# erizmr/SPH_Taichi

Measured on AMD Instinct MI355X. Metric: WCSPH steps/sec at 1.74 M particles (+ ms/step breakdown sort/neighbour/force), higher is better.
Workload: dtype f32

## Files before the change

### include/sph_hip.h

```cpp
#ifndef SPH_HIP_H
#define SPH_HIP_H

#include <stddef.h>
#include <stdint.h>

#ifdef __cplusplus
extern "C" {
#endif

#define SPH_ABI_VERSION 6

typedef struct SphContext SphContext;

typedef struct SphParams {
    int32_t n_particles;
    int32_t capacity;
    int32_t grid_num[3];
    int32_t cell_origin[3];
    int32_t n_objects;
    int32_t cold_capacity;
    float grid_size;
    float support_radius;
    float particle_diameter;
    float m_V0;
// ... 49 lines not shown
    SPH_OPT_FUSED_STEP = 2,
    SPH_OPT_BRICK_SHAPE = 3,
    SPH_OPT_NO_DYNAMIC_SOLIDS = 4 ,
    SPH_OPT_DEBUG_ABLATE = 5,
    SPH_OPT_SLAB_DROP_OUTSIDE = 6 ,
    SPH_OPT_UNIFORM_FLUID = 7  ,
    SPH_OPT_UNIFORM_FLUID_STATE = 8 ,
    SPH_OPT_SORT_BY_PID = 9    ,
    SPH_OPT_KERNEL_VARIANT = 10 ,
    SPH_OPT_RIGID_BATCH = 11   ,
    SPH_OPT_DF_RUNAHEAD = 13,
    SPH_OPT_EXACT_MATH = 12    ,
    SPH_OPT_RIGID_SUMS_FROM_X0 = 14,
    SPH_OPT_PURE_FLUID_INSTANCE = 15 ,
    SPH_OPT_BRICK_RECORDS = 16 ,
    SPH_OPT_DF_FUSE_ERROR = 17
};
#define SPH_VAR_GROUPS 1
#define SPH_VAR_MFMA 32
#define SPH_VAR_GAT_LDS 2
#define SPH_VAR_GAT_LDS4 4
#define SPH_VAR_FORCE_BF 8
#define SPH_VAR_DEEP 16

typedef struct SphTimings {
    double sort_ms, neighbour_ms, force_ms, integrate_ms, halo_ms, total_ms;
    int64_t steps;
} SphTimings;

int32_t sph_abi_version(void);
int32_t sph_device_count(void);
// ... 154 lines not shown
```

### sph_taichi_amd/_lib.py

```python
from __future__ import annotations

import ctypes as C
import os

from . import build as _build

_F3 = C.c_float * 3
_I3 = C.c_int32 * 3


class SphParams(C.Structure):
    _fields_ = [
        ("n_particles", C.c_int32), ("capacity", C.c_int32), ("grid_num", _I3), ("cell_origin", _I3),
        ("n_objects", C.c_int32), ("cold_capacity", C.c_int32),
        ("grid_size", C.c_float), ("support_radius", C.c_float), ("particle_diameter", C.c_float),
        ("m_V0", C.c_float), ("density_0", C.c_float), ("stiffness", C.c_float), ("exponent", C.c_float),
        ("viscosity", C.c_float), ("surface_tension", C.c_float), ("dt", C.c_float),
        ("g", _F3), ("domain_size", _F3), ("padding", C.c_float), ("wall_hi", _F3),
        ("k_w", C.c_float), ("k_dw", C.c_float), ("visc_d_nu", C.c_float), ("visc_eps", C.c_float),
    ]


class SphTimings(C.Structure):
    _fields_ = [("sort_ms", C.c_double), ("neighbour_ms", C.c_double), ("force_ms", C.c_double),
# ... 20 lines not shown


class SphRenderParams(C.Structure):
    _fields_ = [("width", C.c_int32), ("height", C.c_int32), ("eye", _F3), ("lookat", _F3), ("up", _F3),
                ("fov_y_deg", C.c_float), ("radius", C.c_float), ("near_plane", C.c_float), ("light", _F3),
                ("ambient", C.c_float), ("background", C.c_uint8 * 3), ("draw_box", C.c_uint8),
                ("box_end", _F3), ("box_color", _F3)]


RENDER_MAX_INVISIBLE = 32

F_OBJECT_ID, F_X, F_X_0, F_V, F_ACCELERATION, F_M_V, F_M, F_DENSITY, F_PRESSURE, F_MATERIAL, F_COLOR, \
    F_IS_DYNAMIC, F_GRID_IDS, F_GRID_PARTICLES_NUM, F_PID, F_RIGID_REST_CM, F_DFSPH_FACTOR, F_DENSITY_ADV = range(18)
OPT_GATHER_IMPL, OPT_TIMING, OPT_FUSED_STEP, OPT_BRICK_SHAPE, OPT_NO_DYNAMIC_SOLIDS, OPT_DEBUG_ABLATE, \
    OPT_SLAB_DROP_OUTSIDE, OPT_UNIFORM_FLUID, OPT_UNIFORM_FLUID_STATE, OPT_SORT_BY_PID, OPT_KERNEL_VARIANT, \
    OPT_RIGID_BATCH, OPT_EXACT_MATH, OPT_DF_RUNAHEAD, OPT_RIGID_SUMS_FROM_X0, OPT_PURE_FLUID_INSTANCE, OPT_BRICK_RECORDS, OPT_DF_FUSE_ERROR = range(18)
VAR_GROUPS, VAR_GAT_LDS, VAR_GAT_LDS4, VAR_FORCE_BF, VAR_DEEP, VAR_MFMA = 1, 2, 4, 8, 16, 32
VAR_DEFAULT = VAR_GROUPS | VAR_FORCE_BF | VAR_DEEP

ABI_VERSION = 6

_ctx = C.c_void_p
SYMBOLS = [
    ("sph_abi_version", C.c_int32, []),
    ("sph_device_count", C.c_int32, []),
    ("sph_create", C.c_int32, [C.POINTER(SphParams), C.c_int32, C.c_void_p, C.POINTER(_ctx)]),
    ("sph_destroy", C.c_int32, [_ctx]),
    ("sph_last_error", C.c_char_p, [_ctx]),
    ("sph_set_option", C.c_int32, [_ctx, C.c_int32, C.c_int32]),
    ("sph_get_option", C.c_int32, [_ctx, C.c_int32, C.POINTER(C.c_int32)]),
    ("sph_set_params", C.c_int32, [_ctx, C.POINTER(SphParams)]),
# ... 152 lines not shown
```

### sph_taichi_amd/csrc/sph_api.hip

```cpp
#include <sched.h>
#include "sph_internal.h"

#define SCAN_TILE 2048

int sphk_init_pid(SphContext* c);
int sphk_build_dyn_list(SphContext* c);

static thread_local char g_err[256] = "";

int sph_fail(SphContext* c, int code, const char* what) {
    if (c) snprintf(c->err, sizeof(c->err), "%s", what);
    else snprintf(g_err, sizeof(g_err), "%s", what);
    return code;
}

DevView sph_view(const SphContext* c) {
    DevView d;
    const SphParams& p = c->p;
    d.N = c->N; d.G = c->G;
    d.nx = p.grid_num[0]; d.ny = p.grid_num[1]; d.nz = p.grid_num[2];
    d.tgt_lo = 0; d.tgt_hi = p.grid_num[0]; d.tgt_lo2 = d.tgt_hi2 = 0;
#ifdef SPH_PROFILE
    d.ablate = c->opt_ablate;
    d.prof_ts = (c->opt_ablate & (3 << 28)) ? reinterpret_cast<unsigned long long*>(c->stage) : nullptr;
// ... 5 lines not shown
    d.d2 = p.particle_diameter * p.particle_diameter;
    d.m_V0 = p.m_V0; d.rho0 = p.density_0; d.stiffness = p.stiffness; d.exponent = p.exponent;
    d.exp_int = (p.exponent >= 1.0f && p.exponent <= 32.0f && p.exponent == (float)(int)p.exponent) ? (int)p.exponent : 0;
    d.sigma = p.surface_tension; d.dt = p.dt;
    d.gx = p.g[0]; d.gy = p.g[1]; d.gz = p.g[2];
    d.pad = p.padding;
    d.k_w = p.k_w; d.k_dw = p.k_dw; d.visc_d_nu = p.visc_d_nu; d.visc_eps = p.visc_eps;
    d.w_zero = p.k_w * (6.0f * 0.0f - 6.0f * 0.0f + 1.0f);
    {
        const float q = p.particle_diameter / p.support_radius;
        if (q <= 0.5f) d.w_d = p.k_w * (6.0f * q * q * q - 6.0f * q * q + 1.0f);
        else if (q <= 1.0f) d.w_d = p.k_w * 2.0f * (1.0f - q) * (1.0f - q) * (1.0f - q);
        else d.w_d = 0.0f;
    }
    const int o = c->in_off;
    d.xm = c->xm[c->cur] + o; d.vf = c->vf[c->cur] + o; d.aux = c->aux[c->cur] + o; d.key = c->key[c->cur] + o;
    d.eos = c->eos; d.eos2 = reinterpret_cast<float2*>(c->eos); d.acc = c->acc + o; d.acc_fx = c->acc_fx + 3 * (size_t)o; d.cell_end = c->cell_end;
    d.x0_cold = c->x0_cold; d.rigid_rest_cm = c->rigid_rest_cm; d.polar_fb = c->dyn_count ? c->dyn_count + 3 : nullptr;
    d.m_eps = c->df.m_eps;
    d.stg = c->stg; d.gat = c->gat; d.kbuf = reinterpret_cast<float*>(c->gat);
    d.m_u = c->m_uniform; d.write_sg = 0; d.write_k = 0;
    d.whx = p.wall_hi[0]; d.why = p.wall_hi[1]; d.whz = p.wall_hi[2];
    d.fuse_advect = c->fuse_advect;
    d.df_bpart = c->df_collect ? c->df_bpart : nullptr;
    d.gate = (c->df_epoch && c->opt_df_runahead) ? c->df_gate : nullptr;
    d.gate_epoch = c->df_epoch;
    d.fx_scale = ldexp(1.0, c->rigid_fx_exp);
    d.store_acc = !(c->fuse_advect && c->skip_acc);
    d.rigid_from_x0 = 0;
    return d;
}

__global__ void k_read_layer_offsets(const int* __restrict__ cell_end, const int* __restrict__ layers, int n,
                                     int per_layer, int* __restrict__ out) {
    const int k = blockIdx.x * blockDim.x + threadIdx.x;
    if (k >= n) return;
    const int L = layers[k];
    out[k] = L > 0 ? cell_end[(size_t)L * per_layer - 1] : 0;
// ... 68 lines not shown
    c->tgt_layers[0] = c->tgt_layers[2] = 0;
    c->tgt_layers[1] = c->tgt_layers[3] = params->grid_num[0];
    c->opt_gather_impl = 1;
    c->opt_fused = 1;
    c->opt_timing = 0;
    c->timing_phase = 0;
    c->opt_brick_shape = 0;
    c->opt_rigid_batch = 1;
    c->opt_df_fuse_err = 1;
    c->df_collect = 0;
    c->opt_df_runahead = 0;
    c->opt_exact_math = 0;
    c->opt_rigid_x0 = 0;
    c->opt_pure_instance = 1;
    c->opt_brick_rec = 1;
    if (stream) { c->stream = (hipStream_t)stream; c->own_stream = false; }
    else {
        if (hipStreamCreateWithFlags(&c->stream, hipStreamNonBlocking) != hipSuccess) {
            delete c;
            return sph_fail(nullptr, SPH_E_NO_DEVICE, "hipStreamCreate failed");
        }
        c->own_stream = true;
    }
    const size_t cap = (size_t)c->cap;
    c->scan_blocks = (c->G + 1 + SCAN_TILE - 1) / SCAN_TILE;
    int rc = 0;
    for (int s = 0; s < 2 && !rc; ++s) {
        rc = rc ? rc : alloc_dev(c, (void**)&c->xm[s], cap * 16);
        rc = rc ? rc : alloc_dev(c, (void**)&c->vf[s], cap * 16);
        rc = rc ? rc : alloc_dev(c, (void**)&c->aux[s], cap * 16);
// ... 62 lines not shown
    for (int s = 0; s < SPH_MAX_TIMED_STEPS && !rc; ++s)
        for (int k = 0; k < 5 && !rc; ++k)
            if (hipEventCreate(&c->ev[s][k]) != hipSuccess) rc = SPH_E_NOMEM;
    if (!rc && hipStreamSynchronize(c->stream) != hipSuccess) rc = SPH_E_NO_DEVICE;
    if (rc) {
        snprintf(g_err, sizeof(g_err), "sph_create failed: %s", c->err);
        sph_destroy(c);
        return rc;
    }
    c->n_dyn_host = -1;
    c->rigid_fx_exp = 30;
    sph_invalidate_lists(c);
    c->opt_uniform = -1; c->uniform_state = -1; c->m_uniform = 0.0f;
    c->opt_variant = SPH_VAR_DEFAULT;
    if (const char* e = getenv("SPH_KERNEL_VARIANT")) { const int v = atoi(e) & 31; c->opt_variant = variant_mask_ok(v) ? v : SPH_VAR_DEFAULT; }
    memset(&c->df_stats, 0, sizeof(c->df_stats));
    c->df.enable_divergence_solver = 1; c->df.m_max_iterations_v = 100; c->df.m_max_iterations = 100;
    c->df.fluid_particle_num = 0; c->df.m_eps = 1e-5f; c->df.reserved_ = 0.0f; c->df.max_error_V = 0.1; c->df.max_error = 0.05;
    *out = c;
    return 0;
}

int32_t sph_destroy(SphContext* c) {
    if (!c) return 0;
    (void)hipSetDevice(c->device);
    if (c->stream) (void)hipStreamSynchronize(c->stream);
    void* ptrs[] = {c->xm[0], c->xm[1], c->vf[0], c->vf[1], c->aux[0], c->aux[1], c->key[0], c->key[1], c->eos, c->stg, c->gat, c->acc,
                    c->acc_tmp, c->cell_buf[0], c->cell_buf[1], c->rank_off, c->idx_unstable, c->scan_status, c->x0_cold, c->color_cold,
                    c->rigid_rest_cm, c->dyn_list, c->dyn_count, c->acc_fx, c->rigid_part, c->rigid_R, c->df_err, c->df_part, c->df_bpart, c->stage, c->glist, c->gcnt, c->brick_list, c->brick_count, c->brick_list2, c->brick_count2, c->brick_rec};
    for (void* p : ptrs) if (p) (void)hipFree(p);
// ... 16 lines not shown

int32_t sph_set_option(SphContext* c, int32_t option, int32_t value) {
    if (!c) return SPH_E_INVALID;
    switch (option) {
        case SPH_OPT_GATHER_IMPL: if (value < 0 || value > 1) return sph_fail(c, SPH_E_INVALID, "gather impl must be 0 or 1"); c->opt_gather_impl = value; c->uniform_state = -1; return 0;
        case SPH_OPT_TIMING: c->opt_timing = value > 0 ? value : 0; c->timing_phase = 0; return 0;
        case SPH_OPT_FUSED_STEP: c->opt_fused = value ? 1 : 0; return 0;
        case SPH_OPT_BRICK_SHAPE: if (value < 0 || value > 1) return sph_fail(c, SPH_E_INVALID, "brick shape must be 0 (adaptive height) or 1 (fixed 4x2x4)"); c->opt_brick_shape = value; sph_invalidate_lists(c); return 0;
        case SPH_OPT_NO_DYNAMIC_SOLIDS: c->opt_no_dynamic = value ? 1 : 0; c->n_dyn_host = -1; c->uniform_state = -1; return 0;
        case SPH_OPT_DEBUG_ABLATE:
#ifndef SPH_PROFILE
            if (value != 0) return sph_fail(c, SPH_E_INVALID, "section ablation exists only in the profiling build (python -m sph_taichi_amd.build --profile; bench.py --ablate loads it)");
#endif
            c->opt_ablate = value;
            return 0;
        case SPH_OPT_SLAB_DROP_OUTSIDE: c->opt_drop_outside = value ? 1 : 0; c->uniform_state = -1; return 0;
        case SPH_OPT_SORT_BY_PID: c->opt_sort_by_pid = value ? 1 : 0; return 0;
        case SPH_OPT_RIGID_BATCH: c->opt_rigid_batch = value ? 1 : 0; return 0;
        case SPH_OPT_EXACT_MATH: c->opt_exact_math = value ? 1 : 0; sph_invalidate_lists(c); return 0;
        case SPH_OPT_DF_RUNAHEAD: c->opt_df_runahead = value ? 1 : 0; return 0;
        case SPH_OPT_KERNEL_VARIANT:
            if (value < -1 || value > 63 || (value > 0 && !variant_mask_ok(value))) return sph_fail(c, SPH_E_INVALID, "kernel variant must be -1 (default) or a mask of SPH_VAR_* (GAT_LDS and GAT_LDS4 exclude each other)");
            c->opt_variant = value < 0 ? SPH_VAR_DEFAULT : value;
            sph_invalidate_lists(c);
            return 0;
        case SPH_OPT_UNIFORM_FLUID: if (value < -1 || value > 1) return sph_fail(c, SPH_E_INVALID, "uniform-fluid option must be -1, 0 or 1"); c->opt_uniform = value; c->uniform_state = -1; return 0;
        case SPH_OPT_RIGID_SUMS_FROM_X0: c->opt_rigid_x0 = value ? 1 : 0; return 0;
        case SPH_OPT_PURE_FLUID_INSTANCE:
            if (value < 0 || value > 2) return sph_fail(c, SPH_E_INVALID, "pure-fluid instance option must be 0, 1 or 2");
            c->opt_pure_instance = value; sph_invalidate_lists(c); return 0;
        case SPH_OPT_BRICK_RECORDS: c->opt_brick_rec = value ? 1 : 0; sph_invalidate_lists(c); return 0;
        case SPH_OPT_DF_FUSE_ERROR: c->opt_df_fuse_err = value ? 1 : 0; return 0;
    }
    return sph_fail(c, SPH_E_INVALID, "unknown option");
}

int32_t sph_get_option(const SphContext* c, int32_t option, int32_t* value) {
    if (!c || !value) return SPH_E_INVALID;
    switch (option) {
        case SPH_OPT_GATHER_IMPL: *value = c->opt_gather_impl; return 0;
        case SPH_OPT_TIMING: *value = c->opt_timing; return 0;
        case SPH_OPT_FUSED_STEP: *value = c->opt_fused; return 0;
        case SPH_OPT_BRICK_SHAPE: *value = c->opt_brick_shape; return 0;
        case SPH_OPT_NO_DYNAMIC_SOLIDS: *value = c->opt_no_dynamic; return 0;
        case SPH_OPT_DEBUG_ABLATE: *value = c->opt_ablate; return 0;
        case SPH_OPT_SLAB_DROP_OUTSIDE: *value = c->opt_drop_outside; return 0;
        case SPH_OPT_UNIFORM_FLUID: *value = c->opt_uniform; return 0;
        case SPH_OPT_SORT_BY_PID: *value = c->opt_sort_by_pid; return 0;
        case SPH_OPT_RIGID_BATCH: *value = c->opt_rigid_batch; return 0;
        case SPH_OPT_EXACT_MATH: *value = (c->opt_exact_math && c->uniform_state != 0) ? 1 : 0; return 0;
        case SPH_OPT_KERNEL_VARIANT: *value = c->opt_variant; return 0;
        case SPH_OPT_DF_RUNAHEAD: *value = c->opt_df_runahead; return 0;
        case SPH_OPT_UNIFORM_FLUID_STATE: *value = c->uniform_state; return 0;
        case SPH_OPT_RIGID_SUMS_FROM_X0: *value = c->opt_rigid_x0; return 0;
        case SPH_OPT_PURE_FLUID_INSTANCE: *value = c->opt_pure_instance; return 0;
        case SPH_OPT_BRICK_RECORDS: *value = c->opt_brick_rec; return 0;
        case SPH_OPT_DF_FUSE_ERROR: *value = c->opt_df_fuse_err; return 0;
    }
    return SPH_E_INVALID;
}

int32_t sph_set_params(SphContext* c, const SphParams* p) {
    if (!c || !p) return SPH_E_INVALID;
    if (p->capacity != c->p.capacity || p->n_objects != c->p.n_objects || p->cold_capacity != c->p.cold_capacity ||
        memcmp(p->grid_num, c->p.grid_num, sizeof(p->grid_num)) != 0 ||
        memcmp(p->cell_origin, c->p.cell_origin, sizeof(p->cell_origin)) != 0)
        return sph_fail(c, SPH_E_INVALID, "sph_set_params: sizes differ from sph_create");
    const int n = c->p.n_particles;
    c->p = *p;
    c->p.n_particles = n;
    return 0;
}

int32_t sph_set_dt(SphContext* c, float dt) {
    if (!c) return SPH_E_INVALID;
    c->p.dt = dt;
    return 0;
}

int32_t sph_set_particle_count(SphContext* c, int32_t n) {
    if (!c || n < 0 || n > c->cap) return sph_fail(c, SPH_E_INVALID, "particle count out of range");
    c->N = n;
    c->n_dyn_host = -1;
    sph_forget_pure_fluid(c);
    sphd_set_changed(c->dv);
// ... 235 lines not shown
    c->ev_used = 0;
    return 0;
}

static int uniform_fluid(SphContext* c) {
    if (c->opt_uniform == 0 || c->opt_gather_impl != 1 || (c->opt_drop_outside && !c->opt_no_dynamic)) {
        c->uniform_state = 0;
        return 0;
    }
    if (c->uniform_state >= 0) return 0;
    return sphk_check_uniform_fluid(c);
}

static int step_sweeps(SphContext* c, hipEvent_t* ev, const int32_t* dynamic_ids, int32_t n_dynamic) {
    int rc = 0;
    bool fused_advect = false;
    if (c->n_dyn_host > 0) { rc = sphk_gather(c, GM_BVOL_DYNAMIC); if (rc) return rc; }
    if (c->opt_fused) {
        rc = uniform_fluid(c);
        rc = rc ? rc : sphk_gather(c, GM_DENSITY_EOS);
        if (rc) return rc;
        if (ev) SPH_HIP(c, hipEventRecord(ev[2], c->stream));
        const bool fuse = c->uniform_state == 1 && sphd_one_gather_wcsph(c->dv) && !c->opt_drop_outside &&
                          c->opt_gather_impl == 1 && c->N > 0;
        c->fuse_advect = fuse ? 1 : 0;
        rc = sphk_gather(c, GM_FORCE_FUSED);
        c->fuse_advect = 0;
        if (rc) return rc;
        fused_advect = fuse;
    } else {
        rc = sphk_gather(c, GM_DENSITY);
        if (rc) return rc;
        if (ev) SPH_HIP(c, hipEventRecord(ev[2], c->stream));
        rc = sphk_gather(c, GM_NONPRESSURE);
        rc = rc ? rc : sphk_eos(c);
        rc = rc ? rc : sphk_gather(c, GM_PRESSURE);
        if (rc) return rc;
    }
    if (ev) SPH_HIP(c, hipEventRecord(ev[3], c->stream));
    if (fused_advect) return sphk_rigid_solve_all(c, dynamic_ids, n_dynamic, true);
    rc = sphk_advect(c, true);
    if (rc) return rc;
    if (c->n_dyn_host > 0) { rc = sphk_rigid_solve_all(c, dynamic_ids, n_dynamic, false); if (rc) return rc; }
    return 0;
}

int32_t sph_set_target_layers(SphContext* c, int32_t dlo, int32_t dhi, int32_t flo, int32_t fhi) {
    if (!c) return SPH_E_INVALID;
    const int nx = c->p.grid_num[0];
    if (dlo < 0 || dhi > nx || dlo > dhi || flo < 0 || fhi > nx || flo > fhi) return sph_fail(c, SPH_E_INVALID, "sph_set_target_layers: bad range");
    c->tgt_layers[0] = dlo; c->tgt_layers[1] = dhi; c->tgt_layers[2] = flo; c->tgt_layers[3] = fhi;
    return 0;
}

int32_t sph_slab_set_window(SphContext* c, int32_t origin_x, int32_t nx) {
// ... 149 lines not shown
    ENTER(c);
    if (first < 0 || count < 0 || first + count > c->in_off + c->N) return sph_fail(c, SPH_E_INVALID, "sph_select_range: out of range");
    c->in_off += first;
    c->N = count;
    sph_forget_pure_fluid(c);
    sphd_set_changed(c->dv);
    c->have_keys = c->have_prefix = c->sorted = false;
    c->n_dyn_host = -1;
    return 0;
}

int32_t sph_truncate(SphContext* c, int32_t n) {
    if (!c || n < 0 || n > c->N) return sph_fail(c, SPH_E_INVALID, "sph_truncate: out of range");
    if (n != c->N && !c->opt_no_dynamic) c->n_dyn_host = -1;
    if (n != c->N) sph_forget_pure_fluid(c);
    c->N = n;
    return 0;
}

int32_t sph_pack_range(SphContext* c, int32_t first, int32_t count, void* dst) {
    ENTER(c);
    if (first < 0 || count < 0 || first + count > c->N || (count > 0 && !dst)) return sph_fail(c, SPH_E_INVALID, "sph_pack_range: out of range");
    if (count == 0) return 0;
    const size_t b = (size_t)count * 16, o = (size_t)c->in_off + first;
    char* d = (char*)dst;
    SPH_HIP(c, hipMemcpyAsync(d, c->xm[c->cur] + o, b, hipMemcpyDeviceToDevice, c->stream));
    SPH_HIP(c, hipMemcpyAsync(d + b, c->vf[c->cur] + o, b, hipMemcpyDeviceToDevice, c->stream));
    SPH_HIP(c, hipMemcpyAsync(d + 2 * b, c->aux[c->cur] + o, b, hipMemcpyDeviceToDevice, c->stream));
    return 0;
}
// ... 409 lines not shown
```

### sph_taichi_amd/csrc/sph_derived.h

```cpp
#pragma once

struct SphPartKey {
    int id;
    int lo, hi, lo2, hi2;
    bool operator==(const SphPartKey& o) const { return id == o.id && lo == o.lo && hi == o.hi && lo2 == o.lo2 && hi2 == o.hi2; }
    bool inside(const SphPartKey& o) const {
        const bool in1 = lo >= o.lo && hi <= o.hi;
        const bool in2 = lo2 == hi2 || (lo2 >= o.lo && hi2 <= o.hi);
        return id == o.id && o.lo2 == o.hi2 && in1 && in2;
    }
};

enum SphPartHit { SPH_PART_NO = 0, SPH_PART_SUBSET = 1, SPH_PART_EXACT = 2 };

struct SphDerived {
    bool lists_valid;
    bool gcnt_written;
    int stg_kind;
    int k_kind;
    bool bricks_valid;
    SphPartKey bricks_key;
    bool brec_valid;
    SphPartKey brec_key;
    bool df_bpart_valid;
    bool aux_stale;
    bool brick_count_zero;
};

static inline void sphd_invalidate(SphDerived& s) { s.lists_valid = s.bricks_valid = s.brec_valid = false; s.stg_kind = s.k_kind = 0; }
static inline void sphd_set_changed(SphDerived& s) { sphd_invalidate(s); s.aux_stale = false; }
static inline void sphd_sorted(SphDerived& s, bool built, const SphPartKey& key) {
    sphd_set_changed(s);
    s.gcnt_written = false;
    s.brick_count_zero = false;
    s.bricks_valid = built;
    if (built) s.bricks_key = key;
}
static inline void sphd_partition_rebuilt(SphDerived& s, const SphPartKey& key) {
    s.lists_valid = s.brec_valid = false;
    s.brick_count_zero = false;
    s.bricks_valid = true;
    s.bricks_key = key;
}
static inline void sphd_lists_written(SphDerived& s, int stg_kind) {
    s.lists_valid = s.gcnt_written = true;
    s.stg_kind = stg_kind;
    s.k_kind = 0;
    if (stg_kind == 1) s.aux_stale = true;
}
static inline void sphd_records_written(SphDerived& s, const SphPartKey& key) { s.brec_valid = true; s.brec_key = key; }
static inline void sphd_k_written(SphDerived& s, int kind) { s.k_kind = kind; }
static inline void sphd_bpart_written(SphDerived& s) { s.df_bpart_valid = true; }
static inline void sphd_bpart_consumed(SphDerived& s) { s.df_bpart_valid = false; }
static inline void sphd_aux_folded(SphDerived& s) { s.aux_stale = false; }
static inline void sphd_count_zeroed(SphDerived& s, bool zero) { s.brick_count_zero = zero; }

static inline SphPartHit sphd_partition_hit(const SphDerived& s, const SphPartKey& key) {
    if (!s.bricks_valid) return SPH_PART_NO;
    return key == s.bricks_key ? SPH_PART_EXACT : key.inside(s.bricks_key) ? SPH_PART_SUBSET : SPH_PART_NO;
}
static inline bool sphd_lists_usable(const SphDerived& s) { return s.lists_valid; }
static inline bool sphd_records_usable(const SphDerived& s, const SphPartKey& key) { return s.lists_valid && s.brec_valid && key == s.brec_key; }
static inline bool sphd_one_gather_wcsph(const SphDerived& s) { return s.lists_valid && s.stg_kind == 1; }
static inline bool sphd_one_gather_df(const SphDerived& s, int k_kind) { return s.lists_valid && s.stg_kind == 2 && s.k_kind == k_kind; }
static inline bool sphd_stats_have_lists(const SphDerived& s) { return s.gcnt_written; }
static inline bool sphd_bpart_ready(const SphDerived& s) { return s.df_bpart_valid; }
static inline bool sphd_aux_in_eos2(const SphDerived& s) { return s.aux_stale; }
static inline bool sphd_count_is_zero(const SphDerived& s) { return s.brick_count_zero; }
```

### sph_taichi_amd/csrc/sph_gather.hip

```cpp
#include "sph_internal.h"
#include "sph_bricks.h"

#define TPB 256

#ifdef SPH_PROFILE
#define SPH_ABL(d_, m_) ((d_).ablate & (m_))
#define SPH_TS(slot_)                                                                                         \
    do {                                                                                                      \
        if (ts_on && threadIdx.x == 0) d.prof_ts[(size_t)blockIdx.x * 8 + (slot_)] = wall_clock64();          \
    } while (0)
#else
#define SPH_ABL(d_, m_) 0
#define SPH_TS(slot_) do { } while (0)
#endif

struct Target {
    float x, y, z, mV;
    float vx, vy, vz;
    int flags;
    float m, rho, p, dpi;
    float s0;
    float ax, ay, az;
    float px, py, pz;
    float st_c;
// ... 454 lines not shown
            d.acc[i] = a;
        }
        return;
    }
    if (MODE == GM_FORCE_FUSED || MODE == GM_FORCE_FUSED_U) {
        if (gathered) {
            const float4 a = make_float4(t.ax + t.px, t.ay + t.py, t.az + t.pz, 0.f);
            if (MODE != GM_FORCE_FUSED_U || d.store_acc) d.acc[i] = a;
            if (MODE == GM_FORCE_FUSED_U && d.fuse_advect) {
                float4 xm = make_float4(t.x, t.y, t.z, t.mV);
                float4 vf = make_float4(t.vx, t.vy, t.vz, __int_as_float(t.flags));
                const float hi[3] = {d.whx, d.why, d.whz};
                advect_one<true>(d, hi, xm, vf, a);
                d.xm[i] = xm;
                d.vf[i] = vf;
            }
        }
        return;
    }
}

template <int MODE>
__device__ __forceinline__ float4 load_C_global(const DevView& d, int j) {
    if (MODE == GM_FORCE_FUSED || mode_is_df_iter<MODE>() || MODE == GM_DF_NONPRESSURE) return d.eos[j];
    if (MODE == GM_NONPRESSURE || MODE == GM_PRESSURE) return make_C_from_aux<MODE>(d.aux[j]);
    return make_float4(0.f, 0.f, 0.f, 0.f);
}

template <int MODE>
__device__ __forceinline__ void gather_walk_global(const DevView& d, Target& t, int i) {
// ... 263 lines not shown
    const int total = sColS[64];
    if (T == 0) {
        if (mode_is_df_vdiv<MODE>() && d.df_bpart != nullptr && tid == 0) d.df_bpart[bidx] = 0.0;
        return;
    }
#ifdef SPH_PROFILE
    if (ts_on && threadIdx.x == 0) d.prof_ts[(size_t)blockIdx.x * 8 + 6] = ((unsigned long long)(unsigned)T << 32) | (unsigned)total;
#endif
    const bool overflow = total > CFG::CAP;

    auto tmap = [&](int tn) -> int {
        if (mode_reads_list<MODE>() || V_MFMA || (tn | 31) >= T) return tn;
        const int l = tn & 31;
        return (tn & ~31) | (int)(((0x73261540u >> ((l >> 2) * 4)) & 7u) << 2) | (l & 3);
    };
    int col_0 = 0, gi_0 = 0, key_0 = 0;
    float4 Ai_0 = make_float4(0.f, 0.f, 0.f, 0.f), Bi_0 = Ai_0, Ei_0 = Ai_0;
    if (V_MFMA || tid < T) {
        const int tq = tmap(V_MFMA ? min(tid, T - 1) : tid);
#pragma unroll
        for (int step = 16; step > 0; step >>= 1)
            if (sTOff[col_0 + step] <= tq) col_0 += step;
        gi_0 = sTG[col_0] + (tq - sTOff[col_0]);
        if (!(MODE == GM_FORCE_FUSED_U && !overflow)) Ai_0 = d.xm[gi_0];
        Bi_0 = d.vf[gi_0];
        Ei_0 = target_load_E<MODE>(d, gi_0);
        if (!mode_reads_list<MODE>()) key_0 = d.key[gi_0];
    }

    if (!overflow) {
        float4 buf[CFG::PER];
        float4 bufg[V_GLDS ? CFG::PER : 1];
        (void)bufg;
#pragma unroll
// ... 31 lines not shown
                const float xl = buf[u].x - Ox, yl = buf[u].y - Oy, zl = buf[u].z - Oz;
                if (HAS_W) {
                    sQ[idx] = make_float4(-2.0f * xl, -2.0f * yl, -2.0f * zl, xl * xl + yl * yl + zl * zl);
                    if (!V_PURE) sW[idx] = buf[u].w;
                } else {
                    sQ[idx] = buf[u];
                    if (V_GLDS) sG[idx] = bufg[u];
                }
            }
        }
    }
    __syncthreads();
    SPH_TS(2);

    double df_errsum = 0.0;
    for (int tn = tid; V_MFMA ? (tn & ~63) < T : tn < T; tn += TPB) {
        const bool valid = !V_MFMA || tn < T;
        int col = col_0, gi = gi_0, key_i = key_0;
        float4 Ai = Ai_0, Bi = Bi_0, Ei = Ei_0;
        if (tn != tid) {
            const int tq = tmap(V_MFMA ? min(tn, T - 1) : tn);
            col = 0;
#pragma unroll
            for (int step = 16; step > 0; step >>= 1)
                if (sTOff[col + step] <= tq) col += step;
            gi = sTG[col] + (tq - sTOff[col]);
            if (!(MODE == GM_FORCE_FUSED_U && !overflow)) Ai = d.xm[gi];
            Bi = d.vf[gi];
            Ei = target_load_E<MODE>(d, gi);
            if (!mode_reads_list<MODE>()) key_i = d.key[gi];
        }
        const int li = gi - sColG[col];
        if (MODE == GM_FORCE_FUSED_U && !overflow) {
            if (li >= sColS[col]) {
                Ai = sQ[li];
                Ai.w = Ai.w > 0.0f ? d.m_V0 : -Ai.w;
// ... 340 lines not shown
                    if (k + 1 < cnt) pair(s1);
                    fetch(s0, nxt.x & 0xffffu);
                    if (k + 2 < cnt) pair(s2);
                    fetch(s1, nxt.x >> 16);
                    if (k + 3 < cnt) pair(s3);
                    cur = nxt; nxt = nn;
                }
            }
        }
        if (walk) {
            target_init<mode_walk<MODE>()>(d, t, Ai, Bi, Ei);
            gather_walk_global<mode_walk<MODE>()>(d, t, gi);
        }
        SPH_TS(3);
        if (valid) target_finish<MODE, V_EXACT>(d, t, gi, g, Ei);
        if (mode_is_df_vdiv<MODE>() && d.df_bpart != nullptr) df_errsum += (double)t.df_err;
    }
    SPH_TS(4);
    if constexpr (mode_is_df_vdiv<MODE>()) {
        __shared__ double df_red[TPB / 64];
        if (d.df_bpart != nullptr) {
#pragma unroll
            for (int off = 32; off > 0; off >>= 1) df_errsum += __shfl_down(df_errsum, off, 64);
            if (lane == 0) df_red[wave] = df_errsum;
            __syncthreads();
            if (tid == 0) {
                double tot = 0.0;
                for (int w = 0; w < TPB / 64; ++w) tot += df_red[w];
                d.df_bpart[bidx] = tot;
            }
// ... 398 lines not shown
```

### sph_taichi_amd/csrc/sph_internal.h

```cpp
#pragma once
#include <hip/hip_runtime.h>
#include <stdint.h>
#include <stdio.h>
#include <string.h>

#include "../../include/sph_hip.h"
#include "sph_derived.h"

#define SPH_MATERIAL_SOLID 0
#define SPH_MATERIAL_FLUID 1
#define SPH_MAX_TIMED_STEPS 128
#define SPH_GLIST_ROWS 96
#define SPH_DF_ERR_BLOCKS 512
#define SPH_VAR_PURE_INTERNAL 64
#define SPH_VAR_DEFAULT (SPH_VAR_GROUPS | SPH_VAR_FORCE_BF | SPH_VAR_DEEP)

struct DevView {
    int N, G;
    int nx, ny, nz;
    int ox, oy, oz;
    int tgt_lo, tgt_hi;
    int tgt_lo2, tgt_hi2;
    int sort_by_pid;
    int drop_outside;
// ... 7 lines not shown
#endif
    float grid_size, h, inv_h, d2, m_V0, rho0, stiffness, exponent, sigma, dt;
    float gx, gy, gz;
    float pad;
    float k_w, k_dw, visc_d_nu, visc_eps;
    float w_zero, w_d;
    float m_eps;
    float m_u;
    double fx_scale;
    float whx, why, whz;
    int fuse_advect;
    int write_sg;
    int write_k;
    int store_acc;
    int rigid_from_x0;
    float4* xm;
    float4* vf;
    float4* aux;
    float4* eos;
    float2* eos2;
    float4* stg;
    float4* gat;
    float* kbuf;
    float4* acc;
    long long* acc_fx;
    int* key;
    int* cell_end;
    const float* x0_cold;
    int* polar_fb;
    float* rigid_rest_cm;
// ... 20 lines not shown
    bool use_side;
    int2* brick_list2;
    int* brick_count2;
    int off_zero_mask;
    int off_stamp;
    bool off_stamp_pending;
    bool off_in_sort;
    CellIdx16 off_ix;
    int tgt_layers[4];
    int nx_alloc;
    int in_off;
    float4* xm[2];
    float4* vf[2];
    float4* aux[2];
    int* key[2];
    float4* eos;
    float2* eos2;
    float4* stg;
    float4* gat;
    float4* acc;
    float4* acc_tmp;
    long long* acc_fx;
    int* cell_end;
    int* cell_buf[2];
    int cell_cur;
    bool next_cells_zero;
    int* rank_off;
    int* idx_unstable;
    unsigned long long* scan_status;
    unsigned scan_epoch;
    int* scan_err;
    unsigned short* glist;
    int glist_shift;
    unsigned char* gcnt;
    int4* brick_rec;
    int opt_brick_rec;
    int2* brick_list;
    int* brick_count;
    int brick_cap;
    int scan_blocks;
    float* x0_cold;
    int* color_cold;
    float* rigid_rest_cm;
    int* dyn_list;
    int* dyn_count;
    int n_dyn_host;
    int rigid_fx_exp;
    double* rigid_part;
    int rigid_part_blocks;
    float* rigid_R;
    void* stage;
// ... 118 lines not shown
__device__ __forceinline__ int sph_flags_object(int f) { return (int)((unsigned)f >> 9); }
__device__ __forceinline__ bool sph_is_fluid(int f) { return (f & 0xFF) == SPH_MATERIAL_FLUID; }
__device__ __forceinline__ bool sph_is_static_rigid(int f) { return (f & 0x1FF) == 0; }
__device__ __forceinline__ bool sph_is_dynamic_rigid(int f) { return (f & 0x1FF) == 0x100; }

__device__ __forceinline__ int sph_cell_coord(float p, float grid_size, int origin, int n) {
    int c = (int)(p / grid_size) - origin;
    c = c < 0 ? 0 : c;
    c = c > n - 1 ? n - 1 : c;
    return c;
}
__device__ __forceinline__ int sph_flatten(const DevView& d, int cx, int cy, int cz) {
    return (cx * d.ny + cy) * d.nz + cz;
}

__device__ __forceinline__ int sph_wave_inclusive_scan(int v, int lane) {
#pragma unroll
    for (int off = 1; off < 64; off <<= 1) {
        int n = __shfl_up(v, off, 64);
        if (lane >= off) v += n;
    }
    return v;
}

template <bool FAST>
__device__ __forceinline__ float sph_tait_pow(const DevView& d, float x) {
    if (d.exp_int > 0) {
        float r = 1.0f, b = x;
        for (int e = d.exp_int; e; e >>= 1) {
            if (e & 1) r *= b;
// ... 40 lines not shown
```

### sph_taichi_amd/csrc/sph_sort.hip

```cpp
#include "sph_internal.h"
#include "sph_bricks.h"

#define TPB 256
#define SCAN_IPT 8
#define SCAN_TILE (TPB * SCAN_IPT)

__global__ __launch_bounds__(TPB) void k_hash_histogram(DevView d, int* __restrict__ cell_cnt,
                                                        int* __restrict__ rank_off, int* __restrict__ brick_count) {
    const int i = blockIdx.x * TPB + threadIdx.x;
    const int lane = threadIdx.x & 63;
    if (i == 0) brick_count[0] = brick_count[1] = 0;
    int c = -1 - lane;
    if (i < d.N) {
        const float4 p = d.xm[i];
        const int cx = sph_cell_coord(p.x, d.grid_size, d.ox, d.nx);
        const int cy = sph_cell_coord(p.y, d.grid_size, d.oy, d.ny);
        const int cz = sph_cell_coord(p.z, d.grid_size, d.oz, d.nz);
        c = sph_flatten(d, cx, cy, cz);
        if (d.drop_outside) {
            const int raw = (int)(p.x / d.grid_size) - d.ox;
            if (raw < 0 || raw >= d.nx) c = d.G;
        }
        d.key[i] = c;
    }
    const int prev = __shfl_up(c, 1, 64);
    const bool head = (lane == 0) || (prev != c);
    const unsigned long long heads = __ballot(head);
    const unsigned long long below = heads & (~0ull >> (63 - lane));
    const int head_lane = 63 - __clzll(below);
    const unsigned long long above = (head_lane == 63) ? 0ull : (heads >> (head_lane + 1));
    const int run_len = above ? (__ffsll((long long)above)) : (64 - head_lane);
    int base = 0;
    if (head && c >= 0) base = atomicAdd(&cell_cnt[c], run_len);
    base = __shfl(base, head_lane, 64);
    if (i < d.N) rank_off[i] = base + (lane - head_lane);
}

__device__ __forceinline__ int block_exclusive_offset(int thread_total, int* s_wave, int& block_total) {
    const int lane = threadIdx.x & 63, wave = threadIdx.x >> 6;
    const int incl = sph_wave_inclusive_scan(thread_total, lane);
    if (lane == 63) s_wave[wave] = incl;
    __syncthreads();
    int wave_off = 0, tot = 0;
#pragma unroll
    for (int w = 0; w < TPB / 64; ++w) {
        const int s = s_wave[w];
        if (w < wave) wave_off += s;
        tot += s;
    }
    block_total = tot;
    return wave_off + incl - thread_total;
}

#define SCAN_SPIN_LIMIT (1 << 22)
__global__ __launch_bounds__(TPB) void k_scan_fused(int4* __restrict__ data, unsigned long long* __restrict__ status,
                                                    unsigned epoch, int* __restrict__ err) {
    __shared__ int s_wave[TPB / 64];
    const int base = (blockIdx.x * TPB + threadIdx.x) * (SCAN_IPT / 4);
    int4 v[SCAN_IPT / 4];
    int t = 0;
#pragma unroll
    for (int k = 0; k < SCAN_IPT / 4; ++k) {
        v[k] = data[base + k];
        t += v[k].x + v[k].y + v[k].z + v[k].w;
    }
    int tot;
    const int ex = block_exclusive_offset(t, s_wave, tot);
    if (threadIdx.x == 0)
        __hip_atomic_store(&status[blockIdx.x], ((unsigned long long)epoch << 32) | (unsigned)tot, __ATOMIC_RELAXED,
                           __HIP_MEMORY_SCOPE_AGENT);
    int before = 0;
    for (int j = threadIdx.x; j < (int)blockIdx.x; j += TPB) {
// ... 89 lines not shown
    if (!live) return;
    const int dst = b + rank;
    const float4 xm = d.xm[i];
    const float4 vf = d.vf[i];
    const float4 aux = d.aux[i];
    xm_out[dst] = xm;
    vf_out[dst] = vf;
    aux_out[dst] = aux;
    key_out[dst] = c;
    if (SORT_ACC) acc_out[dst] = d.acc[i];
    if (c != d.G && sph_is_dynamic_rigid(__float_as_int(vf.w))) dyn_list[atomicAdd(dyn_count, 1)] = dst;
}

int sphk_hash_histogram(SphContext* c) {
    const int Gpad = c->scan_blocks * SCAN_TILE;
    int* nxt = c->cell_buf[c->cell_cur ^ 1];
    if (!c->next_cells_zero) SPH_HIP(c, hipMemsetAsync(nxt, 0, sizeof(int) * (size_t)Gpad, c->stream));
    c->cell_cur ^= 1;
    c->cell_end = nxt;
    c->next_cells_zero = false;
    sphd_count_zeroed(c->dv, c->N > 0);
    if (c->N > 0) {
        DevView d = sph_view(c);
        hipLaunchKernelGGL(k_hash_histogram, dim3((c->N + TPB - 1) / TPB), dim3(TPB), 0, c->stream, d, c->cell_end,
                           c->rank_off, c->brick_count);
        SPH_LAUNCH_CHECK(c);
    }
    return 0;
}

int sphk_scan(SphContext* c) {
    const int nb = c->scan_blocks;
    c->scan_epoch += 1u;
    if (c->scan_epoch == 0u) {
        SPH_HIP(c, hipMemsetAsync(c->scan_status, 0, (size_t)(nb + 1) * 8, c->stream));
        c->scan_epoch = 1u;
    }
    hipLaunchKernelGGL(k_scan_fused, dim3(nb), dim3(TPB), 0, c->stream, (int4*)c->cell_end, c->scan_status, c->scan_epoch,
                       c->scan_err);
    SPH_LAUNCH_CHECK(c);
    return 0;
}

int sphk_sort_scatter(SphContext* c, bool sort_acc) {
    if (c->N <= 0) return 0;
    DevView d = sph_view(c);
    const int nb = (c->N + TPB - 1) / TPB;
    const int o = c->cur ^ 1;
    int4* zero_dst = reinterpret_cast<int4*>(c->cell_buf[c->cell_cur ^ 1]);
    const int zero_n4 = c->scan_blocks * SCAN_TILE / 4;
    BrickListArgs bl;
    SphPartKey bl_key;
    int rc = sphk_brick_list_prepare(c, &bl, &bl_key);
    if (rc) return rc;
    if (bl.nblocks > 0 && !sphd_count_is_zero(c->dv)) {
        SPH_HIP(c, hipMemsetAsync(c->brick_count, 0, 2 * sizeof(int), c->stream));
    }
    CellIdx16 off_ix;
    int* off_out = nullptr;
    for (int k = 0; k < 16; ++k) off_ix.v[k] = -1;
    if (c->off_in_sort) {
        off_ix = c->off_ix;
        SPH_HIP(c, hipHostGetDevicePointer((void**)&off_out, c->h_pinned, 0));
    }
    if (c->off_in_sort) {
        c->off_stamp = c->off_stamp == 0x7fffffff ? 1 : c->off_stamp + 1;
        c->off_stamp_pending = true;
    }
    hipLaunchKernelGGL(k_unstable_place, dim3(nb), dim3(TPB), 0, c->stream, d, c->rank_off, c->idx_unstable, c->dyn_count, off_ix, off_out,
                       c->off_stamp);
    SPH_LAUNCH_CHECK(c);
    if (sort_acc)
        hipLaunchKernelGGL(k_stable_scatter<true>, dim3(nb + bl.nblocks), dim3(TPB), bl.lds_bytes, c->stream, d, c->idx_unstable, c->xm[o],
                           c->vf[o], c->aux[o], c->key[o], c->acc_tmp, c->dyn_list, c->dyn_count, zero_dst, zero_n4, bl);
    else
        hipLaunchKernelGGL(k_stable_scatter<false>, dim3(nb + bl.nblocks), dim3(TPB), bl.lds_bytes, c->stream, d, c->idx_unstable, c->xm[o],
                           c->vf[o], c->aux[o], c->key[o], c->acc_tmp, c->dyn_list, c->dyn_count, zero_dst, zero_n4, bl);
    SPH_LAUNCH_CHECK(c);
    c->next_cells_zero = true;
    c->cur = o;
    sphd_sorted(c->dv, bl.nblocks > 0, bl_key);
    if (sort_acc) {
        float4* t = c->acc;
        c->acc = c->acc_tmp;
        c->acc_tmp = t;
    }
    return 0;
}
```

Measured before the change: 2185.

## Compute next-step cell hash inside fused force/advect kernel, skip histogram launch

When the fused force+advect path runs on a pure-fluid instance, each target thread now hashes its freshly advected position into the next cell-count buffer and next key buffer. The following step's histogram kernel is then skipped, and the brick counter reset moves into the scan kernel. A separate key double-buffer index is added so the ahead-written keys do not clobber the keys still being read, and several invalidation hooks drop the precomputed hash when parameters or counts change. The intent is to remove one full pass over particle positions and a kernel launch per step. In exchange, the force kernel gains per-wave atomics and ballots and must run whole-wave rounds, which adds state-tracking complexity.

After: 2178. Within noise of the previous version (-0.4%).

```diff
diff --git a/include/sph_hip.h b/include/sph_hip.h
--- a/include/sph_hip.h
+++ b/include/sph_hip.h
@@ -87,7 +87,8 @@
     SPH_OPT_RIGID_SUMS_FROM_X0 = 14,
     SPH_OPT_PURE_FLUID_INSTANCE = 15 ,
     SPH_OPT_BRICK_RECORDS = 16 ,
-    SPH_OPT_DF_FUSE_ERROR = 17
+    SPH_OPT_DF_FUSE_ERROR = 17 ,
+    SPH_OPT_HASH_AHEAD = 18
 };
 #define SPH_VAR_GROUPS 1
 #define SPH_VAR_MFMA 32
diff --git a/sph_taichi_amd/_lib.py b/sph_taichi_amd/_lib.py
--- a/sph_taichi_amd/_lib.py
+++ b/sph_taichi_amd/_lib.py
@@ -58,7 +58,7 @@
     F_IS_DYNAMIC, F_GRID_IDS, F_GRID_PARTICLES_NUM, F_PID, F_RIGID_REST_CM, F_DFSPH_FACTOR, F_DENSITY_ADV = range(18)
 OPT_GATHER_IMPL, OPT_TIMING, OPT_FUSED_STEP, OPT_BRICK_SHAPE, OPT_NO_DYNAMIC_SOLIDS, OPT_DEBUG_ABLATE, \
     OPT_SLAB_DROP_OUTSIDE, OPT_UNIFORM_FLUID, OPT_UNIFORM_FLUID_STATE, OPT_SORT_BY_PID, OPT_KERNEL_VARIANT, \
-    OPT_RIGID_BATCH, OPT_EXACT_MATH, OPT_DF_RUNAHEAD, OPT_RIGID_SUMS_FROM_X0, OPT_PURE_FLUID_INSTANCE, OPT_BRICK_RECORDS, OPT_DF_FUSE_ERROR = range(18)
+    OPT_RIGID_BATCH, OPT_EXACT_MATH, OPT_DF_RUNAHEAD, OPT_RIGID_SUMS_FROM_X0, OPT_PURE_FLUID_INSTANCE, OPT_BRICK_RECORDS, OPT_DF_FUSE_ERROR, OPT_HASH_AHEAD = range(19)
 VAR_GROUPS, VAR_GAT_LDS, VAR_GAT_LDS4, VAR_FORCE_BF, VAR_DEEP, VAR_MFMA = 1, 2, 4, 8, 16, 32
 VAR_DEFAULT = VAR_GROUPS | VAR_FORCE_BF | VAR_DEEP
 
diff --git a/sph_taichi_amd/csrc/sph_api.hip b/sph_taichi_amd/csrc/sph_api.hip
--- a/sph_taichi_amd/csrc/sph_api.hip
+++ b/sph_taichi_amd/csrc/sph_api.hip
@@ -43,7 +43,7 @@
         else d.w_d = 0.0f;
     }
     const int o = c->in_off;
-    d.xm = c->xm[c->cur] + o; d.vf = c->vf[c->cur] + o; d.aux = c->aux[c->cur] + o; d.key = c->key[c->cur] + o;
+    d.xm = c->xm[c->cur] + o; d.vf = c->vf[c->cur] + o; d.aux = c->aux[c->cur] + o; d.key = c->key[c->key_cur] + o;
     d.eos = c->eos; d.eos2 = reinterpret_cast<float2*>(c->eos); d.acc = c->acc + o; d.acc_fx = c->acc_fx + 3 * (size_t)o; d.cell_end = c->cell_end;
     d.x0_cold = c->x0_cold; d.rigid_rest_cm = c->rigid_rest_cm; d.polar_fb = c->dyn_count ? c->dyn_count + 3 : nullptr;
     d.m_eps = c->df.m_eps;
@@ -51,6 +51,8 @@
     d.m_u = c->m_uniform; d.write_sg = 0; d.write_k = 0;
     d.whx = p.wall_hi[0]; d.why = p.wall_hi[1]; d.whz = p.wall_hi[2];
     d.fuse_advect = c->fuse_advect;
+    d.hash_ahead = c->hash_ahead;
+    d.key_next = c->key[c->key_cur ^ 1] + o; d.cell_next = c->cell_buf[c->cell_cur ^ 1]; d.rank_off = c->rank_off;
     d.df_bpart = c->df_collect ? c->df_bpart : nullptr;
     d.gate = (c->df_epoch && c->opt_df_runahead) ? c->df_gate : nullptr;
     d.gate_epoch = c->df_epoch;
@@ -149,6 +151,7 @@
     c->opt_rigid_x0 = 0;
     c->opt_pure_instance = 1;
     c->opt_brick_rec = 1;
+    c->opt_hash_ahead = 1;
     if (stream) { c->stream = (hipStream_t)stream; c->own_stream = false; }
     else {
         if (hipStreamCreateWithFlags(&c->stream, hipStreamNonBlocking) != hipSuccess) {
@@ -241,6 +244,7 @@
     c->opt_uniform = -1; c->uniform_state = -1; c->m_uniform = 0.0f;
     c->opt_variant = SPH_VAR_DEFAULT;
     if (const char* e = getenv("SPH_KERNEL_VARIANT")) { const int v = atoi(e) & 31; c->opt_variant = variant_mask_ok(v) ? v : SPH_VAR_DEFAULT; }
+    if (const char* e = getenv("SPH_DISABLE_HASH_AHEAD")) { if (atoi(e) != 0) c->opt_hash_ahead = 0; }
     memset(&c->df_stats, 0, sizeof(c->df_stats));
     c->df.enable_divergence_solver = 1; c->df.m_max_iterations_v = 100; c->df.m_max_iterations = 100;
     c->df.fluid_particle_num = 0; c->df.m_eps = 1e-5f; c->df.reserved_ = 0.0f; c->df.max_error_V = 0.1; c->df.max_error = 0.05;
@@ -287,7 +291,7 @@
 #endif
             c->opt_ablate = value;
             return 0;
-        case SPH_OPT_SLAB_DROP_OUTSIDE: c->opt_drop_outside = value ? 1 : 0; c->uniform_state = -1; return 0;
+        case SPH_OPT_SLAB_DROP_OUTSIDE: c->opt_drop_outside = value ? 1 : 0; c->uniform_state = -1; sphd_hash_dropped(c->dv); return 0;
         case SPH_OPT_SORT_BY_PID: c->opt_sort_by_pid = value ? 1 : 0; return 0;
         case SPH_OPT_RIGID_BATCH: c->opt_rigid_batch = value ? 1 : 0; return 0;
         case SPH_OPT_EXACT_MATH: c->opt_exact_math = value ? 1 : 0; sph_invalidate_lists(c); return 0;
@@ -304,6 +308,7 @@
             c->opt_pure_instance = value; sph_invalidate_lists(c); return 0;
         case SPH_OPT_BRICK_RECORDS: c->opt_brick_rec = value ? 1 : 0; sph_invalidate_lists(c); return 0;
         case SPH_OPT_DF_FUSE_ERROR: c->opt_df_fuse_err = value ? 1 : 0; return 0;
+        case SPH_OPT_HASH_AHEAD: c->opt_hash_ahead = value ? 1 : 0; sphd_hash_dropped(c->dv); return 0;
     }
     return sph_fail(c, SPH_E_INVALID, "unknown option");
 }
@@ -329,6 +334,7 @@
         case SPH_OPT_PURE_FLUID_INSTANCE: *value = c->opt_pure_instance; return 0;
         case SPH_OPT_BRICK_RECORDS: *value = c->opt_brick_rec; return 0;
         case SPH_OPT_DF_FUSE_ERROR: *value = c->opt_df_fuse_err; return 0;
+        case SPH_OPT_HASH_AHEAD: *value = (c->opt_hash_ahead && sphd_hash_is_ahead(c->dv)) ? 1 : 0; return 0;
     }
     return SPH_E_INVALID;
 }
@@ -342,6 +348,7 @@
     const int n = c->p.n_particles;
     c->p = *p;
     c->p.n_particles = n;
+    sphd_hash_dropped(c->dv);
     return 0;
 }
 
@@ -607,7 +614,7 @@
 
 static int step_sweeps(SphContext* c, hipEvent_t* ev, const int32_t* dynamic_ids, int32_t n_dynamic) {
     int rc = 0;
-    bool fused_advect = false;
+    bool fused_advect = false, hashed_ahead = false;
     if (c->n_dyn_host > 0) { rc = sphk_gather(c, GM_BVOL_DYNAMIC); if (rc) return rc; }
     if (c->opt_fused) {
         rc = uniform_fluid(c);
@@ -616,11 +623,17 @@
         if (ev) SPH_HIP(c, hipEventRecord(ev[2], c->stream));
         const bool fuse = c->uniform_state == 1 && sphd_one_gather_wcsph(c->dv) && !c->opt_drop_outside &&
                           c->opt_gather_impl == 1 && c->N > 0;
+        const bool ahead = fuse && c->opt_hash_ahead && c->pure_fluid && c->pure_fluid_n == c->N && c->opt_pure_instance != 2 &&
+                           c->in_off == 0 && c->next_cells_zero;
         c->fuse_advect = fuse ? 1 : 0;
+        c->hash_ahead = ahead ? 1 : 0;
+        if (ahead) c->next_cells_zero = false;
         rc = sphk_gather(c, GM_FORCE_FUSED);
         c->fuse_advect = 0;
+        c->hash_ahead = 0;
         if (rc) return rc;
         fused_advect = fuse;
+        hashed_ahead = ahead;
     } else {
         rc = sphk_gather(c, GM_DENSITY);
         if (rc) return rc;
@@ -631,7 +644,11 @@
         if (rc) return rc;
     }
     if (ev) SPH_HIP(c, hipEventRecord(ev[3], c->stream));
-    if (fused_advect) return sphk_rigid_solve_all(c, dynamic_ids, n_dynamic, true);
+    if (fused_advect) {
+        rc = sphk_rigid_solve_all(c, dynamic_ids, n_dynamic, true);
+        if (!rc && hashed_ahead) sphd_hashed_ahead(c->dv);
+        return rc;
+    }
     rc = sphk_advect(c, true);
     if (rc) return rc;
     if (c->n_dyn_host > 0) { rc = sphk_rigid_solve_all(c, dynamic_ids, n_dynamic, false); if (rc) return rc; }
@@ -811,6 +828,7 @@
     if (!c || n < 0 || n > c->N) return sph_fail(c, SPH_E_INVALID, "sph_truncate: out of range");
     if (n != c->N && !c->opt_no_dynamic) c->n_dyn_host = -1;
     if (n != c->N) sph_forget_pure_fluid(c);
+    if (n != c->N) sphd_hash_dropped(c->dv);
     c->N = n;
     return 0;
 }
diff --git a/sph_taichi_amd/csrc/sph_derived.h b/sph_taichi_amd/csrc/sph_derived.h
--- a/sph_taichi_amd/csrc/sph_derived.h
+++ b/sph_taichi_amd/csrc/sph_derived.h
@@ -25,9 +25,11 @@
     bool df_bpart_valid;
     bool aux_stale;
     bool brick_count_zero;
+    bool hash_valid;
+    bool count_reset_owed;
 };
 
-static inline void sphd_invalidate(SphDerived& s) { s.lists_valid = s.bricks_valid = s.brec_valid = false; s.stg_kind = s.k_kind = 0; }
+static inline void sphd_invalidate(SphDerived& s) { s.lists_valid = s.bricks_valid = s.brec_valid = s.hash_valid = false; s.stg_kind = s.k_kind = 0; }
 static inline void sphd_set_changed(SphDerived& s) { sphd_invalidate(s); s.aux_stale = false; }
 static inline void sphd_sorted(SphDerived& s, bool built, const SphPartKey& key) {
     sphd_set_changed(s);
@@ -53,7 +55,10 @@
 static inline void sphd_bpart_written(SphDerived& s) { s.df_bpart_valid = true; }
 static inline void sphd_bpart_consumed(SphDerived& s) { s.df_bpart_valid = false; }
 static inline void sphd_aux_folded(SphDerived& s) { s.aux_stale = false; }
-static inline void sphd_count_zeroed(SphDerived& s, bool zero) { s.brick_count_zero = zero; }
+static inline void sphd_count_zeroed(SphDerived& s, bool zero) { s.brick_count_zero = zero; s.count_reset_owed = false; }
+static inline void sphd_hashed_ahead(SphDerived& s) { s.hash_valid = true; }
+static inline void sphd_hash_dropped(SphDerived& s) { s.hash_valid = false; }
+static inline void sphd_hash_consumed(SphDerived& s) { s.hash_valid = false; s.count_reset_owed = true; }
 
 static inline SphPartHit sphd_partition_hit(const SphDerived& s, const SphPartKey& key) {
     if (!s.bricks_valid) return SPH_PART_NO;
@@ -67,3 +72,5 @@
 static inline bool sphd_bpart_ready(const SphDerived& s) { return s.df_bpart_valid; }
 static inline bool sphd_aux_in_eos2(const SphDerived& s) { return s.aux_stale; }
 static inline bool sphd_count_is_zero(const SphDerived& s) { return s.brick_count_zero; }
+static inline bool sphd_hash_is_ahead(const SphDerived& s) { return s.hash_valid; }
+static inline bool sphd_count_reset_owed(const SphDerived& s) { return s.count_reset_owed; }
diff --git a/sph_taichi_amd/csrc/sph_gather.hip b/sph_taichi_amd/csrc/sph_gather.hip
--- a/sph_taichi_amd/csrc/sph_gather.hip
+++ b/sph_taichi_amd/csrc/sph_gather.hip
@@ -492,6 +492,7 @@
                 advect_one<true>(d, hi, xm, vf, a);
                 d.xm[i] = xm;
                 d.vf[i] = vf;
+                t.x = xm.x; t.y = xm.y; t.z = xm.z;
             }
         }
         return;
@@ -785,10 +786,11 @@
         const int l = tn & 31;
         return (tn & ~31) | (int)(((0x73261540u >> ((l >> 2) * 4)) & 7u) << 2) | (l & 3);
     };
+    const bool wave_rounds = V_MFMA || (MODE == GM_FORCE_FUSED_U && d.hash_ahead != 0);
     int col_0 = 0, gi_0 = 0, key_0 = 0;
     float4 Ai_0 = make_float4(0.f, 0.f, 0.f, 0.f), Bi_0 = Ai_0, Ei_0 = Ai_0;
-    if (V_MFMA || tid < T) {
-        const int tq = tmap(V_MFMA ? min(tid, T - 1) : tid);
+    if (wave_rounds || tid < T) {
+        const int tq = tmap(wave_rounds ? min(tid, T - 1) : tid);
 #pragma unroll
         for (int step = 16; step > 0; step >>= 1)
             if (sTOff[col_0 + step] <= tq) col_0 += step;
@@ -850,12 +852,12 @@
     SPH_TS(2);
 
     double df_errsum = 0.0;
-    for (int tn = tid; V_MFMA ? (tn & ~63) < T : tn < T; tn += TPB) {
-        const bool valid = !V_MFMA || tn < T;
+    for (int tn = tid; wave_rounds ? (tn & ~63) < T : tn < T; tn += TPB) {
+        const bool valid = !wave_rounds || tn < T;
         int col = col_0, gi = gi_0, key_i = key_0;
         float4 Ai = Ai_0, Bi = Bi_0, Ei = Ei_0;
         if (tn != tid) {
-            const int tq = tmap(V_MFMA ? min(tn, T - 1) : tn);
+            const int tq = tmap(wave_rounds ? min(tn, T - 1) : tn);
             col = 0;
 #pragma unroll
             for (int step = 16; step > 0; step >>= 1)
@@ -1226,6 +1228,8 @@
         }
         SPH_TS(3);
         if (valid) target_finish<MODE, V_EXACT>(d, t, gi, g, Ei);
+        if (MODE == GM_FORCE_FUSED_U && d.hash_ahead != 0)
+            sph_hash_particle(d, g, gi, make_float4(t.x, t.y, t.z, 0.f), d.key_next, d.cell_next, d.rank_off);
         if (mode_is_df_vdiv<MODE>() && d.df_bpart != nullptr) df_errsum += (double)t.df_err;
     }
     SPH_TS(4);
diff --git a/sph_taichi_amd/csrc/sph_internal.h b/sph_taichi_amd/csrc/sph_internal.h
--- a/sph_taichi_amd/csrc/sph_internal.h
+++ b/sph_taichi_amd/csrc/sph_internal.h
@@ -45,6 +45,10 @@
     int write_k;
     int store_acc;
     int rigid_from_x0;
+    int hash_ahead;
+    int* key_next;
+    int* cell_next;
+    int* rank_off;
     float4* xm;
     float4* vf;
     float4* aux;
@@ -95,6 +99,7 @@
     float4* vf[2];
     float4* aux[2];
     int* key[2];
+    int key_cur;
     float4* eos;
     float2* eos2;
     float4* stg;
@@ -116,6 +121,8 @@
     unsigned char* gcnt;
     int4* brick_rec;
     int opt_brick_rec;
+    int opt_hash_ahead;
+    int hash_ahead;
     int2* brick_list;
     int* brick_count;
     int brick_cap;
@@ -264,6 +271,34 @@
     return (cx * d.ny + cy) * d.nz + cz;
 }
 
+__device__ __forceinline__ void sph_hash_particle(const DevView& d, bool live, int i, const float4 p, int* __restrict__ key,
+                                                  int* __restrict__ cell_cnt, int* __restrict__ rank_off) {
+    const int lane = threadIdx.x & 63;
+    int c = -1 - lane;
+    if (live) {
+        const int cx = sph_cell_coord(p.x, d.grid_size, d.ox, d.nx);
+        const int cy = sph_cell_coord(p.y, d.grid_size, d.oy, d.ny);
+        const int cz = sph_cell_coord(p.z, d.grid_size, d.oz, d.nz);
+        c = sph_flatten(d, cx, cy, cz);
+        if (d.drop_outside) {
+            const int raw = (int)(p.x / d.grid_size) - d.ox;
+            if (raw < 0 || raw >= d.nx) c = d.G;
+        }
+        key[i] = c;
+    }
+    const int prev = __shfl_up(c, 1, 64);
+    const bool head = (lane == 0) || (prev != c);
+    const unsigned long long heads = __ballot(head);
+    const unsigned long long below = heads & (~0ull >> (63 - lane));
+    const int head_lane = 63 - __clzll(below);
+    const unsigned long long above = (head_lane == 63) ? 0ull : (heads >> (head_lane + 1));
+    const int run_len = above ? (__ffsll((long long)above)) : (64 - head_lane);
+    int base = 0;
+    if (head && c >= 0) base = atomicAdd(&cell_cnt[c], run_len);
+    base = __shfl(base, head_lane, 64);
+    if (live) rank_off[i] = base + (lane - head_lane);
+}
+
 __device__ __forceinline__ int sph_wave_inclusive_scan(int v, int lane) {
 #pragma unroll
     for (int off = 1; off < 64; off <<= 1) {
diff --git a/sph_taichi_amd/csrc/sph_sort.hip b/sph_taichi_amd/csrc/sph_sort.hip
--- a/sph_taichi_amd/csrc/sph_sort.hip
+++ b/sph_taichi_amd/csrc/sph_sort.hip
@@ -8,32 +8,11 @@
 __global__ __launch_bounds__(TPB) void k_hash_histogram(DevView d, int* __restrict__ cell_cnt,
                                                         int* __restrict__ rank_off, int* __restrict__ brick_count) {
     const int i = blockIdx.x * TPB + threadIdx.x;
-    const int lane = threadIdx.x & 63;
     if (i == 0) brick_count[0] = brick_count[1] = 0;
-    int c = -1 - lane;
-    if (i < d.N) {
-        const float4 p = d.xm[i];
-        const int cx = sph_cell_coord(p.x, d.grid_size, d.ox, d.nx);
-        const int cy = sph_cell_coord(p.y, d.grid_size, d.oy, d.ny);
-        const int cz = sph_cell_coord(p.z, d.grid_size, d.oz, d.nz);
-        c = sph_flatten(d, cx, cy, cz);
-        if (d.drop_outside) {
-            const int raw = (int)(p.x / d.grid_size) - d.ox;
-            if (raw < 0 || raw >= d.nx) c = d.G;
-        }
-        d.key[i] = c;
-    }
-    const int prev = __shfl_up(c, 1, 64);
-    const bool head = (lane == 0) || (prev != c);
-    const unsigned long long heads = __ballot(head);
-    const unsigned long long below = heads & (~0ull >> (63 - lane));
-    const int head_lane = 63 - __clzll(below);
-    const unsigned long long above = (head_lane == 63) ? 0ull : (heads >> (head_lane + 1));
-    const int run_len = above ? (__ffsll((long long)above)) : (64 - head_lane);
-    int base = 0;
-    if (head && c >= 0) base = atomicAdd(&cell_cnt[c], run_len);
-    base = __shfl(base, head_lane, 64);
-    if (i < d.N) rank_off[i] = base + (lane - head_lane);
+    const bool live = i < d.N;
+    float4 p = make_float4(0.f, 0.f, 0.f, 0.f);
+    if (live) p = d.xm[i];
+    sph_hash_particle(d, live, i, p, d.key, cell_cnt, rank_off);
 }
 
 __device__ __forceinline__ int block_exclusive_offset(int thread_total, int* s_wave, int& block_total) {
@@ -54,8 +33,9 @@
 
 #define SCAN_SPIN_LIMIT (1 << 22)
 __global__ __launch_bounds__(TPB) void k_scan_fused(int4* __restrict__ data, unsigned long long* __restrict__ status,
-                                                    unsigned epoch, int* __restrict__ err) {
+                                                    unsigned epoch, int* __restrict__ err, int* __restrict__ brick_count) {
     __shared__ int s_wave[TPB / 64];
+    if (brick_count != nullptr && blockIdx.x == 0 && threadIdx.x == 0) brick_count[0] = brick_count[1] = 0;
     const int base = (blockIdx.x * TPB + threadIdx.x) * (SCAN_IPT / 4);
     int4 v[SCAN_IPT / 4];
     int t = 0;
@@ -175,6 +155,13 @@
 
 int sphk_hash_histogram(SphContext* c) {
     const int Gpad = c->scan_blocks * SCAN_TILE;
+    if (sphd_hash_is_ahead(c->dv)) {
+        c->cell_cur ^= 1;
+        c->cell_end = c->cell_buf[c->cell_cur];
+        c->key_cur ^= 1;
+        sphd_hash_consumed(c->dv);
+        return 0;
+    }
     int* nxt = c->cell_buf[c->cell_cur ^ 1];
     if (!c->next_cells_zero) SPH_HIP(c, hipMemsetAsync(nxt, 0, sizeof(int) * (size_t)Gpad, c->stream));
     c->cell_cur ^= 1;
@@ -197,9 +184,11 @@
         SPH_HIP(c, hipMemsetAsync(c->scan_status, 0, (size_t)(nb + 1) * 8, c->stream));
         c->scan_epoch = 1u;
     }
+    const bool reset = sphd_count_reset_owed(c->dv);
     hipLaunchKernelGGL(k_scan_fused, dim3(nb), dim3(TPB), 0, c->stream, (int4*)c->cell_end, c->scan_status, c->scan_epoch,
-                       c->scan_err);
+                       c->scan_err, reset ? c->brick_count : nullptr);
     SPH_LAUNCH_CHECK(c);
+    if (reset) sphd_count_zeroed(c->dv, true);
     return 0;
 }
 
@@ -207,7 +196,7 @@
     if (c->N <= 0) return 0;
     DevView d = sph_view(c);
     const int nb = (c->N + TPB - 1) / TPB;
-    const int o = c->cur ^ 1;
+    const int o = c->cur ^ 1, ko = c->key_cur ^ 1;
     int4* zero_dst = reinterpret_cast<int4*>(c->cell_buf[c->cell_cur ^ 1]);
     const int zero_n4 = c->scan_blocks * SCAN_TILE / 4;
     BrickListArgs bl;
@@ -233,13 +222,14 @@
     SPH_LAUNCH_CHECK(c);
     if (sort_acc)
         hipLaunchKernelGGL(k_stable_scatter<true>, dim3(nb + bl.nblocks), dim3(TPB), bl.lds_bytes, c->stream, d, c->idx_unstable, c->xm[o],
-                           c->vf[o], c->aux[o], c->key[o], c->acc_tmp, c->dyn_list, c->dyn_count, zero_dst, zero_n4, bl);
+                           c->vf[o], c->aux[o], c->key[ko], c->acc_tmp, c->dyn_list, c->dyn_count, zero_dst, zero_n4, bl);
     else
         hipLaunchKernelGGL(k_stable_scatter<false>, dim3(nb + bl.nblocks), dim3(TPB), bl.lds_bytes, c->stream, d, c->idx_unstable, c->xm[o],
-                           c->vf[o], c->aux[o], c->key[o], c->acc_tmp, c->dyn_list, c->dyn_count, zero_dst, zero_n4, bl);
+                           c->vf[o], c->aux[o], c->key[ko], c->acc_tmp, c->dyn_list, c->dyn_count, zero_dst, zero_n4, bl);
     SPH_LAUNCH_CHECK(c);
     c->next_cells_zero = true;
     c->cur = o;
+    c->key_cur = ko;
     sphd_sorted(c->dv, bl.nblocks > 0, bl_key);
     if (sort_acc) {
         float4* t = c->acc;
```
